# TencentYoutuResearch/ImageMatching-OETR

Measured on AMD Instinct MI355X. Metric: image-pairs/sec @640x640 (OETR hot path: feature correlation + overlap regression, features resident in HBM), higher is better.
Workload: dtype f32 (3xf16-split operands, fp32 accumulate); 1 GPU; BASELINE configs[1]: batch=8 pairs/GPU, 640x640 -> 20x20 tokens/image, C=256, 8 enc + 2 dec layers, f32_split_f16; pairs_per_gpu=8, global_pairs=8, streams=3, world_size=1, gpu_max_hw_queues=4, encoder_tile_rows=64, tail_mode=direct form (throughput setting for overlapped streams), parallelism=pairs sharded over 1 rank(s); all-gather of boxes only

## Files before the change

imagematching_oetr_amd/csrc/api.hip:

```cpp
#include <math.h>
#include <stdlib.h>
#include <string.h>

#include <string>
#include <vector>

#include "../../include/oetr_hip.h"
#include "common.h"

using namespace oetr;

constexpr int OETR_PREREDUCE_MIN_TOKENS = 768;
constexpr int OETR_DIRECT_TAIL_MIN_ROWS = 16000;

namespace {

thread_local std::string g_err;

oetr_status fail(oetr_status st, const std::string& msg) {
  g_err = msg;
  return st;
}
oetr_status hip_fail(hipError_t e, const char* what) {
  return fail(OETR_ERR_HIP, std::string(what) + ": " + hipGetErrorString(e));
// ... 96 lines not shown
  std::vector<int> kid;
  int used = 0;
  int dropped = 0;
};

struct oetr_ctx {
  oetr_trace* trace = nullptr;
  int device = 0;
  int mode = GM_SPLIT;
  int kv_prereduce = -1;
  mutable int dec_fault = 0;
  int dec_split = 0;
  int tail_mode = 0;
  int policy = 0;
  int enc_tile = 0;
  int attn_full = 0;
  int num_cus = 256;
  float* dev = nullptr;
  size_t dev_floats = 0;
  EncLayerDev enc[OETR_N_ENC];
  DecKVDev dkv;
  DecLayerDev dec[OETR_N_DEC];
  const float* qe[2];
  const float *dec_tgt1, *dec_q0, *dec_qkv1;
  HeadsDev heads;
};

struct oetr_neck_ctx {
  oetr_trace* trace = nullptr;
  int device = 0;
// ... 189 lines not shown

oetr_status run_correlation(oetr_ctx* h, const Geom& g, const Workspace& w, const float* feat1,
                            const float* feat2, const float* pos1, const float* pos2,
                            int enc_layers, hipStream_t s, bool with_decoder = true,
                            bool resident = false, const float* mask1 = nullptr,
                            const float* mask2 = nullptr) {
  EncLaunch p;
  memset(&p, 0, sizeof(p));
  if (!resident) {
    p.feat_nchw[0] = feat1; p.feat_nchw[1] = feat2;
    p.pos_nchw[0] = pos1; p.pos_nchw[1] = pos2;
    p.pos_out = w.pos;
  }
  p.tile_rows = encoder_tile_rows(h, g);
  p.g = encoder_geom(g, p.tile_rows);
#ifdef OETR_ABLATE
  { const char* e = getenv("OETR_ABLATE"); p.dbg = e ? atoi(e) : 0; }
#endif
#ifdef OETR_PHASE_TIMING
  {
    static long long* tb = nullptr;
    if (!tb) (void)hipMalloc(&tb, sizeof(long long) * 16 * 65536);
    p.tbuf = tb;
    g_tbuf = tb;
  }
#endif
  p.x = w.x; p.qp = w.qp; p.pos = w.pos;
  p.mask[0] = mask1; p.mask[1] = mask2;
  p.flags = w.flags;
  p.attn_full = h->attn_full;
// ... 959 lines not shown

void oetr_trace_destroy(oetr_trace_handle t) {
  if (!t) return;
  for (auto& e : t->ev) (void)hipEventDestroy(e);
  delete t;
}

oetr_status oetr_set_encoder_tile(oetr_handle h, int rows) {
  if (!h) return fail(OETR_ERR_BAD_ARG, "oetr_set_encoder_tile: NULL handle");
  if (rows != 0 && rows != TM && rows != 64)
    return fail(OETR_ERR_BAD_ARG, "oetr_set_encoder_tile: rows must be 0 (auto), 32 or 64");
  h->enc_tile = rows;
  return OETR_OK;
}

oetr_status oetr_set_tail_mode(oetr_handle h, int mode) {
  if (!h) return fail(OETR_ERR_BAD_ARG, "oetr_set_tail_mode: NULL handle");
  if (mode < 0 || mode > 3)
    return fail(OETR_ERR_BAD_ARG, "oetr_set_tail_mode: 0 (auto), 1 (P form), 2 (direct form) or 3 (direct form, per-tap staging)");
  if (mode >= 2 && h->mode != GM_SPLIT)
    return fail(OETR_ERR_UNSUPPORTED, "the direct 64-row heat-map conv is built for the two-plane dtypes (F32_SPLIT_F16, F32_SPLIT_QK16)");
  h->tail_mode = mode;
  return OETR_OK;
}

oetr_status oetr_set_decoder_split(oetr_handle h, int k) {
  if (!h) return fail(OETR_ERR_BAD_ARG, "oetr_set_decoder_split: NULL handle");
  if (k != 0 && k != 1 && k != DEC_SPLIT_K)
    return fail(OETR_ERR_BAD_ARG, "oetr_set_decoder_split: 0 (auto), 1 or 4 workgroups per image");
  h->dec_split = k;
// ... 87 lines not shown
```

imagematching_oetr_amd/csrc/common.h:

```cpp
#pragma once
#include <hip/hip_runtime.h>
#include <stdint.h>

#include <type_traits>

namespace oetr {

constexpr int C = 256;
constexpr int NH = 8;
constexpr int HD = 32;
constexpr int FF = 512;
constexpr int TM = 32;
constexpr int LDA = C + 4;
constexpr int LDH = FF + 4;
constexpr int NTHREADS = 256;
constexpr int KV_FLOATS = NH * HD * HD;
constexpr float LN_EPS = 1e-5f;
constexpr float ATTN_EPS = 1e-6f;
constexpr int MAX_TOKENS = 10000;


#ifdef OETR_ABLATE
#define ABL(flags, bit) (((flags) & (bit)) != 0)
#else
// ... 58 lines not shown
constexpr int LDAH = C + 8;
constexpr int LDHH = FF + 8;

struct Geom {
  int N;
  int L[2];
  int hf[2], wf[2];
  int nt[2];
  int row0[2];
  int prow0[2];
  int tile0[2];
  int ntiles;
  int rows;
};

#if defined(__HIPCC__)

__device__ __forceinline__ float wave_max(float v) {
#pragma unroll
  for (int off = 32; off > 0; off >>= 1) v = fmaxf(v, __shfl_xor(v, off, 64));
  return v;
}

__device__ __forceinline__ int crow(int r, int half) {
  return (r & 3) + 8 * (r >> 2) + 4 * half;
}

__device__ __forceinline__ float exp_neg(float x) {
  const float L2E_HI = 1.4426950216293335f, L2E_LO = 1.9259629911266175e-08f;
  const float t = x * L2E_HI;
// ... 724 lines not shown
  float* z0_out;
  float* dkv1_out;
  float* dks1_out;
  const float* dec_q0;
  EncLayerDev b;
  EncLayerDev a;
  DecKVDev d;
  int attn_full;
  const float* kbuf_in;
  const float* vt_in;
  float* kbuf_out;
  float* vt_out;
  int lpad[2];
  size_t vt_off[2];
  int tile_rows;
  int b_cross;
  int kv_reduced;
  int policy;
  int dbg;
  long long* tbuf;
  uint32_t* flags;
  const float* feat_nchw[2];
  const float* pos_nchw[2];
  float* pos_out;
  const float* mask[2];
};

hipError_t launch_encoder(const EncLaunch& p, bool has_b, int tail, int mode, hipStream_t s);
hipError_t launch_kv_reduce(const Geom& g, const float* kvp, const float* ksp, float* kvr, float* ksr,
                            hipStream_t s);
// ... 137 lines not shown
```

imagematching_oetr_amd/csrc/encoder.hip:

```cpp
#include <type_traits>

#include "common.h"


#ifndef OETR_SOAK_AMP
#define OETR_SOAK_AMP 0
#endif
#ifndef OETR_SPLIT_STATE
#define OETR_SPLIT_STATE 1
#endif

namespace oetr {

constexpr int S0_OFF = 0;
constexpr int S1_OFF = S0_OFF + TM * LDA;
constexpr int H_OFF = S1_OFF + TILE_FLOATS;
constexpr int KSUM_OFF = H_OFF + HID_FLOATS;
constexpr int Z_OFF = KSUM_OFF + C;
constexpr int LNP_OFF = Z_OFF + TM * NH;
constexpr int SMEM_FLOATS = LNP_OFF + 6 * C;

template <int NW>
struct EncCfg {
  static constexpr int NT = 8 / NW;
// ... 783 lines not shown
__device__ __forceinline__ void kv_state_write(const f32x16& kv, float ksum, int lane, int wave,
                                               float* __restrict__ kv_out,
                                               float* __restrict__ ks_out, int slot) {
  f32x4* dst = reinterpret_cast<f32x4*>(kv_out) + ((size_t)slot * NH + wave) * 4 * 64;
#pragma unroll
  for (int q = 0; q < 4; ++q) {
    f32x4 o = {kv[4 * q], kv[4 * q + 1], kv[4 * q + 2], kv[4 * q + 3]};
    store16(reinterpret_cast<float*>(dst), (q * 64 + (unsigned)lane) * 16u, o);
  }
  if (lane < 32) (ks_out + (size_t)slot * C + wave * HD)[(unsigned)lane] = ksum;
}

template <bool HAS_B, int TAIL, int MODE, int POL, int ROWS, int RTW = RT, bool MASKED = false>
__device__ __forceinline__ void encoder64_body(const EncLaunch& p, float* smem) {
  constexpr int NMT = RTW / 32, THREADS = 512, TPR = THREADS / RTW, F4 = 64 / TPR;
  using L2 = E2<RTW>;
  using SP = SitePolicy<POL>;
  float* R1f = smem + L2::R1;
  float* R2f = smem + L2::R2;
  Range rg;
  const PlanesT<MODE, RTW> P1(R1f, &rg), P2(R2f, &rg);
  float* Xf = HAS_B ? R2f : R1f;
  float* ksum_s = smem + L2::KSUM;
  float* lnp_s = smem + L2::LNP;
  float* lnx_s = smem + L2::LNX;
  using WS = WStream2T<MODE, ROWS, NMT>;
  WS ws;
  constexpr int P_MERGE = 0;
  constexpr int P_1A = WS::adv(P_MERGE), P_1B = WS::adv(P_1A), P_2A = WS::adv(P_1B), P_2B = WS::adv(P_2A);
  constexpr int P_T0 = HAS_B ? WS::adv(P_2B) : 0;
  constexpr int P_T1 = WS::adv(P_T0), P_T2 = WS::adv(P_T1), P_T3 = WS::adv(P_T2);

  const Geom& g = p.g;
  const int tid = threadIdx.x, lane = tid & 63, wave = __builtin_amdgcn_readfirstlane(tid >> 6);
  const int half = lane >> 5, col = lane & 31;
  const int wcol = 32 * wave;
  const int lrow = tid / TPR, lpart = tid % TPR;

  const int logical = xcd_remap(blockIdx.x, g.ntiles);
  const int per = g.nt[0] + g.nt[1];
  const int n = logical / per;
  const int rem = logical - n * per;
  const int side = rem >= g.nt[0];
  const int t_idx = side ? rem - g.nt[0] : rem;
  const int L = g.L[side];
  const int l0 = t_idx * RTW;
  const int nvalid = min(RTW, L - l0);
  const size_t row_base = (size_t)g.row0[side] + (size_t)n * L + l0;
  const int slot = g.tile0[side] + n * g.nt[side] + t_idx;
  const size_t qrow_base = (size_t)slot * RTW;
  const bool nchw = !HAS_B && p.feat_nchw[0] != nullptr;
  ws.set_rows(nvalid);
  ws.set_lane(lane);

  stage_ln_params<THREADS, HAS_B, TAIL>(lnp_s, p, tid);
  const f32x4* pos = reinterpret_cast<const f32x4*>(
                         p.pos + (size_t)(g.prow0[side] + l0 + min(lrow, nvalid - 1)) * C) + lpart;

  f32x16 xacc[NMT];
  PHASE_STAMP(p, 0);
  if (!HAS_B) PHASE_STAMP(p, 13);

  if (HAS_B) {
    const int ss = p.b_cross ? 1 - side : side;
    const int S_len = g.L[ss];
    const int nts = p.kv_reduced ? 1 : g.nt[ss];
    const int src_slot0 = p.kv_reduced ? ss * g.N + n : g.tile0[ss] + n * g.nt[ss];

    f32x4 kvB[4];
#pragma unroll
    for (int q = 0; q < 4; ++q) kvB[q] = f32x4{0.f, 0.f, 0.f, 0.f};
    {
      constexpr int KVR = 7;
      const unsigned ln = lane, kl = tid & (C - 1);
      const f32x4* kvp = reinterpret_cast<const f32x4*>(p.kv_in) + ((size_t)src_slot0 * NH + wave) * 256;
      const float* ksp = p.ks_in + (size_t)src_slot0 * C;
      float ks = 0.f;
      if (nts == 1) {
#pragma unroll
        for (int e = 0; e < 4; ++e) kvB[e] = kvp[e * 64 + ln];
        ks = ksp[kl];
      } else
      for (int ti0 = 0; ti0 < nts; ti0 += KVR) {
        f32x4 tmp[KVR][4];
        float kt[KVR];
#pragma unroll
        for (int u = 0; u < KVR; ++u) {
          const int ti = min(ti0 + u, nts - 1);
#pragma unroll
          for (int e = 0; e < 4; ++e) tmp[u][e] = kvp[(size_t)ti * (NH * 256) + e * 64 + ln];
          kt[u] = ksp[(size_t)ti * C + kl];
        }
#pragma unroll
        for (int u = 0; u < KVR; ++u)
          if (ti0 + u < nts) {
#pragma unroll
            for (int e = 0; e < 4; ++e) kvB[e] += tmp[u][e];
            ks += kt[u];
          }
      }
      if (tid < C) ksum_s[tid] = ks;
    }
    ws.template prime<C, P_MERGE, SP::MERGE>(p.b.wmerge, p.b.wmerge_l, wave, 0, lane);
    f32x4 qfrag[NMT][4];
    {
      const f32x4* qf = reinterpret_cast<const f32x4*>(p.qp + qrow_base * C) + (size_t)wave * NMT * 4 * 64;
#pragma unroll
      for (int mt = 0; mt < NMT; ++mt)
#pragma unroll
        for (int u = 0; u < 4; ++u) qfrag[mt][u] = qf[(mt * 4 + u) * 64 + (unsigned)lane];
    }
#pragma unroll
    for (int mt = 0; mt < NMT; ++mt) {
      const float* xr = p.x + (row_base + min(32 * mt + col, nvalid - 1)) * C + wcol + 4 * half;
#pragma unroll
      for (int g4 = 0; g4 < 4; ++g4) {
        const f32x4 v = *reinterpret_cast<const f32x4*>(xr + 8 * g4);
#pragma unroll
        for (int i = 0; i < 4; ++i) xacc[mt][4 * g4 + i] = v[i];
      }
    }
    __syncthreads();
    PHASE_STAMP(p, 1);

    {
      f32x4 kvh[2], kvl[2], ksh[2], ksl[2];
      const float inv_S = 1.0f / (float)S_len;
      (void)inv_S;
      if constexpr (gm_f16_range(MODE)) {
#pragma unroll
        for (int s2 = 0; s2 < 2; ++s2) {
          split8(kvB[2 * s2], kvB[2 * s2 + 1], kvh[s2], kvl[s2], rg);
          const float* kr = ksum_s + wave * HD + 4 * half + 16 * s2;
          split8(*reinterpret_cast<const f32x4*>(kr) * inv_S, *reinterpret_cast<const f32x4*>(kr + 8) * inv_S,
                 ksh[s2], ksl[s2], rg);
        }
      }
#pragma unroll
      for (int mt = 0; mt < NMT; ++mt) {
        if (mt == 1 && !ws.two()) break;
        f32x16 macc = {0}, zacc = {0};
        if constexpr (gm_f16_range(MODE)) {
          f32x16 c1 = {0}, cz = {0};
#pragma unroll
          for (int s2 = 0; s2 < 2; ++s2) {
            const f32x4 qh = qfrag[mt][2 * s2], ql = qfrag[mt][2 * s2 + 1];
            mma16_split3(kvh[s2], kvl[s2], qh, ql, macc, c1);
            mma16_split3(ksh[s2], ksl[s2], qh, ql, zacc, cz);
          }
#pragma unroll
          for (int r = 0; r < 16; ++r) macc[r] = fmaf(c1[r], SPLIT_INV, macc[r]);
          zacc[0] = fmaf(cz[0], SPLIT_INV, zacc[0]);
        } else {
#pragma unroll
          for (int ks4 = 0; ks4 < 4; ++ks4) {
            const f32x4 q = qfrag[mt][ks4];
            const f32x4 kk = *reinterpret_cast<const f32x4*>(ksum_s + wave * HD + 4 * half + ks4 * 8);
#pragma unroll
            for (int j = 0; j < 4; ++j) {
              macc = __builtin_amdgcn_mfma_f32_32x32x2f32(kvB[ks4][j], q[j], macc, 0, 0, 0);
              zacc = __builtin_amdgcn_mfma_f32_32x32x2f32(kk[j], q[j], zacc, 0, 0, 0);
            }
          }
        }
        const float zdot = gm_f16_range(MODE) ? zacc[0] * (float)S_len : zacc[0];
        const float zs = (float)S_len / (zdot + ATTN_EPS);
#pragma unroll
        for (int g4 = 0; g4 < 4; ++g4)
          P1.put4(32 * mt + col, wcol + 8 * g4 + 4 * half,
                  f32x4{macc[4 * g4] * zs, macc[4 * g4 + 1] * zs, macc[4 * g4 + 2] * zs, macc[4 * g4 + 3] * zs});
      }
    }
// ... 81 lines not shown
      PHASE_STAMP(p, 7);
      ws.template gemm<FF, P_2B, (TAIL != 2), C, SP::MLP2, SNEXT, XTR>(P1, p.b.w2, p.b.w2_l, wave, 16, lane, xacc,
                                                                       TAIL == 0 ? p.a.wq : p.d.wk[0],
                                                                       TAIL == 0 ? p.a.wq_l : p.d.wk_l[0], wave, 0);
    }
#pragma unroll
    for (int mt = 0; mt < NMT; ++mt)
#pragma unroll
      for (int g4 = 0; g4 < 4; ++g4)
        *reinterpret_cast<f32x4*>(Xf + (32 * mt + col) * LDA + wcol + 8 * g4 + 4 * half) =
            f32x4{xacc[mt][4 * g4], xacc[mt][4 * g4 + 1], xacc[mt][4 * g4 + 2], xacc[mt][4 * g4 + 3]};
    __syncthreads();
#pragma unroll
    for (int i = 0; i < RTW / 8; ++i) {
      const int r = wave + 8 * i;
      if (r < nvalid)
        store16(p.x + (row_base + r) * C, 16u * (unsigned)lane,
                                    *reinterpret_cast<const f32x4*>(Xf + r * LDA + 4 * lane));
    }
    PHASE_STAMP(p, 8);
    if (TAIL == 2) { range_report<MODE>(rg, p.flags); return; }
  } else {
    if (nchw) {
      load_tile_nchw<THREADS, RTW>(R1f, p.feat_nchw[side] + (size_t)n * C * L + l0, L, nvalid, tid);
      load_tile_nchw<THREADS, RTW>(R2f, p.pos_nchw[side] + l0, L, nvalid, tid);
    } else {
#pragma unroll
      for (int i = 0; i < (RTW * C / 4) / THREADS; ++i) {
        const int idx = tid + THREADS * i;
        const int r = idx >> 6, c4 = idx & 63;
        *reinterpret_cast<f32x4*>(R1f + r * LDA + 4 * c4) =
            reinterpret_cast<const f32x4*>(p.x + (row_base + min(r, nvalid - 1)) * C)[c4];
      }
    }
    if (TAIL == 0) ws.template prime<C, P_T0, SP::Q>(p.a.wq, p.a.wq_l, wave, 0, lane);
    if (TAIL == 1) ws.template prime<C, P_T0, SP::DEC_K>(p.d.wk[0], p.d.wk_l[0], wave, 0, lane);
    __syncthreads();
    if (nchw) {
      store_tile_tokens<THREADS, RTW>(p.x + row_base * C, R1f, nvalid, tid);
      if (n == 0) store_tile_tokens<THREADS, RTW>(p.pos_out + (size_t)(g.prow0[side] + l0) * C, R2f, nvalid, tid);
    }
    PHASE_STAMP(p, 14);
  }

  if constexpr (MASKED && TAIL != 2) {
    if (tid < RTW) lnx_s[tid] = tid < nvalid ? p.mask[side][(size_t)n * L + l0 + tid] : 0.f;
  }
  if (TAIL == 0) {
    {
      f32x4 xn[F4], ps[F4];
      if (!HAS_B && nchw) {
        const f32x4* pl = reinterpret_cast<const f32x4*>(R2f + lrow * LDA) + lpart;
#pragma unroll
        for (int i = 0; i < F4; ++i) ps[i] = pl[i * TPR];
      } else {
// ... 9 lines not shown
#pragma unroll
      for (int i = 0; i < F4; ++i) {
        P1.template put4<site_act_lo(SP::Q)>(lrow, 4 * (i * TPR + lpart), (xn[i] * qw[i * TPR] + qb[i * TPR]) + ps[i]);
        P2.template put4<site_act_lo(SP::K) || site_act_lo(SP::V)>(lrow, 4 * (i * TPR + lpart),
                                                                   (xn[i] * kw[i * TPR] + kb[i * TPR]) + ps[i]);
      }
    }
    __syncthreads();
    PHASE_STAMP(p, 9);
    f32x16 accQ[NMT] = {};
    ws.template gemm<C, P_T0, true, C, SP::Q, SP::K, true>(P1, p.a.wq, p.a.wq_l, wave, 0, lane, accQ, p.a.wk,
                                                           p.a.wk_l, wave, 0);
    PHASE_STAMP(p, 10);
    f32x16 accK[NMT] = {}, accV[NMT] = {};
    {
      f32x4* qf = reinterpret_cast<f32x4*>(p.qp + qrow_base * C) + (size_t)wave * NMT * 4 * 64;
      const bool two = ws.two();
      u32x4 qhi = {0, 0, 0, 0}, qlo = {0, 0, 0, 0};
      auto qepi = [&](auto CI_) {
        constexpr int CI = decltype(CI_)::value, mt = NMT == 2 ? CI / 8 : 0, pr = NMT == 2 ? CI % 8 : CI / 2;
        constexpr int s2 = pr / 4, j = pr % 4;
        if constexpr (NMT == 1 && CI % 2 == 1) return;
        if (mt == 1 && !two) return;
        const float qmask = MASKED ? lnx_s[32 * mt + col] : 1.0f;
        const float a = MASKED ? elu1(accQ[mt][2 * pr]) * qmask : elu1(accQ[mt][2 * pr]);
        const float b = MASKED ? elu1(accQ[mt][2 * pr + 1]) * qmask : elu1(accQ[mt][2 * pr + 1]);
        if constexpr (MODE == GM_BF16) {
          if constexpr (pr % 2 == 0) { qhi[0] = __builtin_bit_cast(uint32_t, a); qhi[1] = __builtin_bit_cast(uint32_t, b); }
          else {
            qhi[2] = __builtin_bit_cast(uint32_t, a); qhi[3] = __builtin_bit_cast(uint32_t, b);
            store16(reinterpret_cast<float*>(qf), ((mt * 4 + pr / 2) * 64 + (unsigned)lane) * 16u,
                                        __builtin_bit_cast(f32x4, qhi));
          }
        } else {
          uint32_t h, l;
          cvt_planes2<GM_SPLIT>(a, b, h, l, rg);
          qhi[j] = h; qlo[j] = l;
          if constexpr (j == 3) {
            store16(reinterpret_cast<float*>(qf), ((mt * 4 + 2 * s2) * 64 + (unsigned)lane) * 16u,
                                        __builtin_bit_cast(f32x4, qhi));
            store16(reinterpret_cast<float*>(qf), ((mt * 4 + 2 * s2 + 1) * 64 + (unsigned)lane) * 16u,
                                        __builtin_bit_cast(f32x4, qlo));
          }
        }
      };
      ws.template gemm_epi<C, P_T1, true, C, SP::K, SP::V>(P2, p.a.wk, p.a.wk_l, wave, 0, lane, accK, p.a.wv,
                                                           p.a.wv_l, wave, 0, qepi);
    }
    ws.template gemm<C, P_T2, false, C, SP::V>(P2, p.a.wv, p.a.wv_l, wave, 0, lane, accV, nullptr, nullptr,
                                               0, 0);
    PHASE_STAMP(p, 11);
    f32x16 kv;
    float ksum;
    kv_state_64<MODE, NMT, MASKED>(accK, accV, L, nvalid, half, ws.two(), kv, ksum, rg, lnx_s);
    kv_state_write(kv, ksum, lane, wave, p.kv_out, p.ks_out, slot);
    PHASE_STAMP(p, 12);
  } else if (TAIL == 1) {
    float bias_k[2], bias_v[2];
#pragma unroll
    for (int dl = 0; dl < 2; ++dl) {
      bias_k[dl] = p.d.bk[dl][wcol + col];
      bias_v[dl] = p.d.bv[dl][wcol + col];
    }
    {
      f32x4 xv[F4], ps[F4];
      const f32x4* src = reinterpret_cast<const f32x4*>(Xf + lrow * LDA) + lpart;
#pragma unroll
      for (int i = 0; i < F4; ++i) { xv[i] = src[i * TPR]; ps[i] = pos[i * TPR]; }
      __syncthreads();
#pragma unroll
// ... 3 lines not shown
      }
    }
    __syncthreads();
    auto dec_layer = [&](auto DL) {
      constexpr int dl = decltype(DL)::value;
      constexpr int PK = dl == 0 ? P_T0 : P_T2, PV = dl == 0 ? P_T1 : P_T3;
      f32x16 accK[NMT], accV[NMT];
#pragma unroll
      for (int mt = 0; mt < NMT; ++mt)
#pragma unroll
        for (int r = 0; r < 16; ++r) { accK[mt][r] = bias_k[dl]; accV[mt][r] = bias_v[dl]; }
      ws.template gemm<C, PK, true, C, SP::DEC_K, SP::DEC_V>(P1, p.d.wk[dl], p.d.wk_l[dl], wave, 0, lane, accK,
                                                             p.d.wv[dl], p.d.wv_l[dl], wave, 0);
      ws.template gemm<C, PV, false, C, SP::DEC_V>(P2, p.d.wv[dl], p.d.wv_l[dl], wave, 0, lane, accV, nullptr,
                                                   nullptr, 0, 0);
      f32x16 kv;
      float ksum;
      kv_state_64<MODE, NMT, MASKED>(accK, accV, L, nvalid, half, ws.two(), kv, ksum, rg, lnx_s);
      if constexpr (dl == 1) {
        kv_state_write(kv, ksum, lane, wave, p.dkv1_out, p.dks1_out, slot);
      } else {
        const float* q0 = p.dec_q0 + side * C + wave * HD;
        float a = 0.f;
#pragma unroll
        for (int r = 0; r < 16; ++r) a += q0[crow(r, half)] * kv[r];
        a += __shfl_xor(a, 32, 64);
        float z = q0[col] * ksum;
        z += __shfl_xor(z, 1, 64);
        z += __shfl_xor(z, 2, 64);
        z += __shfl_xor(z, 4, 64);
        z += __shfl_xor(z, 8, 64);
        z += __shfl_xor(z, 16, 64);
        if (half == 0) p.att0_out[(size_t)slot * C + wave * HD + col] = a;
        if (lane == 0) p.z0_out[(size_t)slot * NH + wave] = z;
        ws.template prime<C, P_T2, SP::DEC_K>(p.d.wk[1], p.d.wk_l[1], wave, 0, lane);
      }
    };
    dec_layer(std::integral_constant<int, 0>{});
    dec_layer(std::integral_constant<int, 1>{});
  }
  range_report<MODE>(rg, p.flags);
}

template <bool HAS_B, int TAIL, int MODE, int POL = 0, bool MASKED = false>
__global__ __launch_bounds__(512) void k_encoder64(EncLaunch p) {
  __shared__ __attribute__((aligned(16))) float smem[E2<RT>::SMEM];
  if constexpr (gm_planes(MODE) == 2) {
    const Geom& g = p.g;
    const int logical = xcd_remap(blockIdx.x, g.ntiles);
    const int per = g.nt[0] + g.nt[1];
    const int rem = logical - (logical / per) * per;
    const int side = rem >= g.nt[0];
    const int t_idx = side ? rem - g.nt[0] : rem;
    const int nvalid = min(RT, g.L[side] - t_idx * RT);
    if (__builtin_amdgcn_readfirstlane(nvalid > 32 ? 1 : 0)) encoder64_body<HAS_B, TAIL, MODE, POL, 2, RT, MASKED>(p, smem);
    else encoder64_body<HAS_B, TAIL, MODE, POL, 1, RT, MASKED>(p, smem);
  } else {
    encoder64_body<HAS_B, TAIL, MODE, POL, 0, RT, MASKED>(p, smem);
  }
}

template <bool HAS_B, int TAIL, int MODE, int POL = 0, bool MASKED = false>
__global__ __launch_bounds__(512) void k_encoder32m(EncLaunch p) {
  __shared__ __attribute__((aligned(16))) float smem[E2<TM>::SMEM];
  encoder64_body<HAS_B, TAIL, MODE, POL, 2, TM, MASKED>(p, smem);
}

template <int NOB_TAIL_MAX, class F>
static hipError_t launch_b_tail(bool has_b, int tail, F launch) {
  constexpr std::integral_constant<int, 0> t0{};
// ... 2 lines not shown
  if (has_b) {
    if (tail == 0) launch(std::true_type{}, t0);
    else if (tail == 1) launch(std::true_type{}, t1);
    else launch(std::true_type{}, t2);
  } else {
    if (tail == 0) launch(std::false_type{}, t0);
    else if constexpr (NOB_TAIL_MAX == 0) return hipErrorInvalidValue;
    else if (tail == 1) launch(std::false_type{}, t1);
    else if constexpr (NOB_TAIL_MAX == 1) return hipErrorInvalidValue;
    else launch(std::false_type{}, t2);
  }
  return hipGetLastError();
}

template <int MODE>
static hipError_t launch_encoder_mode(const EncLaunch& p, bool has_b, int tail, hipStream_t s) {
  const dim3 grid(p.g.ntiles);
  if (p.mask[0] || p.mask[1]) {
    if constexpr (MODE == GM_SPLIT) {
      if (!p.mask[0] || !p.mask[1] || (p.policy != 0 && p.policy != 1) || p.attn_full) return hipErrorInvalidValue;
      return launch_b_tail<0>(has_b, tail, [&](auto b, auto t) {
        if (p.policy == 1) {
          if (p.tile_rows == RT) hipLaunchKernelGGL((k_encoder64<b(), t(), MODE, 1, true>), grid, dim3(512), 0, s, p);
          else hipLaunchKernelGGL((k_encoder32m<b(), t(), MODE, 1, true>), grid, dim3(512), 0, s, p);
        } else {
          if (p.tile_rows == RT) hipLaunchKernelGGL((k_encoder64<b(), t(), MODE, 0, true>), grid, dim3(512), 0, s, p);
          else hipLaunchKernelGGL((k_encoder32m<b(), t(), MODE, 0, true>), grid, dim3(512), 0, s, p);
        }
      });
    } else if constexpr (MODE == GM_F32) {
      if (!p.mask[0] || !p.mask[1] || p.policy != 0 || p.attn_full) return hipErrorInvalidValue;
      return launch_b_tail<0>(has_b, tail, [&](auto b, auto t) {
// ... 99 lines not shown
```

imagematching_oetr_amd/hip_engine.py:

```python
import ctypes as C
import os
import time
from pathlib import Path

import torch

_PKG_DIR = Path(__file__).resolve().parent
LIB_PATH = _PKG_DIR / 'csrc' / 'liboetr_hip.so'

N_ENC, N_DEC, D_MODEL, N_HEAD = 8, 2, 256, 8
_f32p = C.POINTER(C.c_float)


class _EncW(C.Structure):
    _fields_ = [(n, _f32p) for n in (
        'q_proj', 'k_proj', 'v_proj', 'merge', 'mlp0', 'mlp2',
        'pre_norm_q_w', 'pre_norm_q_b', 'pre_norm_kv_w', 'pre_norm_kv_b',
        'norm2_w', 'norm2_b')]


class _MhaW(C.Structure):
    _fields_ = [(n, _f32p) for n in (
        'q_proj_w', 'q_proj_b', 'k_proj_w', 'k_proj_b', 'v_proj_w',
        'v_proj_b', 'merge')]
# ... 54 lines not shown
    'oetr_workspace_init', 'oetr_read_flags_async', 'oetr_neck_read_flags_async',
    'oetr_set_state_prereduce', 'oetr_set_tail_mode', 'oetr_set_decoder_split', 'oetr_overlap_frame', 'oetr_read_overlap_image',
    'oetr_forward_masked', 'oetr_feature_correlation_masked', 'oetr_center_estimation_masked',
    'oetr_linear_attention_masked', 'oetr_debug_decoder_fault',
    'oetr_flagslot_device_pointer', 'oetr_forward_flagslot', 'oetr_forward_tokens_flagslot',
    'oetr_neck_forward_tokens_status', 'oetr_debug_mfma_rate')

FLAG_F16_RANGE = 1
FLAG_EXCHANGE = 2
FLAG_INVALID = FLAG_F16_RANGE | FLAG_EXCHANGE
FLAG_PUBLISHED = 0x80000000

BANK_ABI_VERSION = 1
BANK_EXPORTS = ('oetr_bank_abi_version', 'oetr_bank_gather', 'oetr_forward_bank')
FLAG_INDEX = 4

COVIS_ABI_VERSION = 1
COVIS_EXPORTS = ('oetr_covis_abi_version', 'oetr_covis_workspace_bytes', 'oetr_covis_boxes')
COVIS_PARAM_DOUBLES = 40


def hot_path_keys():
    keys = []
    for i in range(N_ENC):
        p = f'transformer.encoder.{i}.'
        keys += [p + s for s in (
            'q_proj.weight', 'k_proj.weight', 'v_proj.weight', 'merge.weight',
            'mlp.0.weight', 'mlp.2.weight', 'pre_norm_q.weight',
            'pre_norm_q.bias', 'pre_norm_kv.weight', 'pre_norm_kv.bias',
            'norm2.weight', 'norm2.bias')]
# ... 151 lines not shown
    lib.oetr_overlap_frame.argtypes = [i, i, i, i] + [C.POINTER(i)] * 4 + [C.POINTER(C.c_double)] * 2
    lib.oetr_read_overlap_image.restype = i
    lib.oetr_read_overlap_image.argtypes = [vp, i, i, i, i, i, i, i, i, i, vp, vp, vp, vp]
    if lib.oetr_abi_version() != ABI_VERSION:
        raise RuntimeError(f'{p}: ABI version {lib.oetr_abi_version()} != '
                           f'{ABI_VERSION}')
    lib.oetr_bank_abi_version.restype = i
    lib.oetr_bank_abi_version.argtypes = []
    bank = [vp, i, vp, vp, i, vp, i]
    lib.oetr_bank_gather.restype = i
    lib.oetr_bank_gather.argtypes = bank + [i, i, vp, vp, vp, vp]
    lib.oetr_forward_bank.restype = i
    lib.oetr_forward_bank.argtypes = [vp] + bank + [i] * 8 + [vp, sz, vp, vp, vp, vp]
    if lib.oetr_bank_abi_version() != BANK_ABI_VERSION:
        raise RuntimeError(f'{p}: bank ABI version {lib.oetr_bank_abi_version()} != {BANK_ABI_VERSION}')
    lib.oetr_covis_abi_version.restype = i
    lib.oetr_covis_abi_version.argtypes = []
    lib.oetr_covis_workspace_bytes.restype = sz
    lib.oetr_covis_workspace_bytes.argtypes = [i]
    lib.oetr_covis_boxes.restype = i
    lib.oetr_covis_boxes.argtypes = [vp, vp, vp, i, i, i, vp, sz] + [vp] * 7
    if lib.oetr_covis_abi_version() != COVIS_ABI_VERSION:
        raise RuntimeError(f'{p}: covis ABI version {lib.oetr_covis_abi_version()} != {COVIS_ABI_VERSION}')
    if path is None:
        _lib = lib
    return lib


class OetrError(RuntimeError):
    pass
# ... 239 lines not shown
        if attention not in self.ATTENTIONS:
            raise ValueError(f'attention must be one of {sorted(self.ATTENTIONS)}')
        self.attention = attention
        if attention != 'linear':
            _check(self.lib, self.lib.oetr_set_attention(self._h, self.ATTENTIONS[attention]),
                   'oetr_set_attention')
        if os.environ.get('OETR_STATE_PREREDUCE'):
            self.set_state_prereduce(int(os.environ['OETR_STATE_PREREDUCE']))

    __del__ = _destructor('oetr_destroy')

    def set_encoder_tile(self, rows):
        _check(self.lib, self.lib.oetr_set_encoder_tile(self._h, int(rows or 0)),
               'oetr_set_encoder_tile')
        self._enc_tile_set = int(rows or 0)

    def _current_ws(self):
        return self._ws.get(torch.cuda.current_stream(self.device).cuda_stream)

    def set_state_prereduce(self, mode):
        _check(self.lib, self.lib.oetr_set_state_prereduce(self._h, int(mode)), 'oetr_set_state_prereduce')

    def set_tail_mode(self, mode):
        _check(self.lib, self.lib.oetr_set_tail_mode(self._h, int(mode)), 'oetr_set_tail_mode')
        self._tail_mode_set = int(mode)

    def set_decoder_split(self, k):
        _check(self.lib, self.lib.oetr_set_decoder_split(self._h, int(k)), 'oetr_set_decoder_split')
        self._dec_split_set = int(k)

# ... 600 lines not shown
```

Measured before the change: 33550 image-pairs/s.

## Pack both images' half-full encoder tail tiles into one mixed workgroup

When both images' last 64-row tiles hold at most 32 valid rows, the two half-tiles now run in one workgroup. A new mixed encoder body (ROWS==3) treats each 32-row half as an independent job, with its own side, slot, KV state and row bounds. This removes one workgroup per pair and keeps the other lanes of the tail tile busy. In exchange it adds a third template instantiation, more index arithmetic and a heavier per-workgroup path for the mixed tile. It is enabled by default only for unmasked, non-full-attention split-f16 runs with 64-row tiles.

```diff
diff --git a/imagematching_oetr_amd/csrc/api.hip b/imagematching_oetr_amd/csrc/api.hip
--- a/imagematching_oetr_amd/csrc/api.hip
+++ b/imagematching_oetr_amd/csrc/api.hip
@@ -6,6 +6,7 @@
 #include <vector>
 
 #include "../../include/oetr_hip.h"
+#include "../../include/oetr_tail_pairing.h"
 #include "common.h"
 
 using namespace oetr;
@@ -134,6 +135,7 @@
   int tail_mode = 0;
   int policy = 0;
   int enc_tile = 0;
+  int tail_pairing = -1;
   int attn_full = 0;
   int num_cus = 256;
   float* dev = nullptr;
@@ -353,6 +355,7 @@
   }
   p.tile_rows = encoder_tile_rows(h, g);
   p.g = encoder_geom(g, p.tile_rows);
+  p.pair_tails = h->tail_pairing != 0;
 #ifdef OETR_ABLATE
   { const char* e = getenv("OETR_ABLATE"); p.dbg = e ? atoi(e) : 0; }
 #endif
@@ -1342,6 +1345,34 @@
   return OETR_OK;
 }
 
+int oetr_tail_pairing_abi_version(void) { return OETR_TAIL_PAIRING_ABI_VERSION; }
+
+oetr_status oetr_set_encoder_tail_pairing(oetr_handle h, int mode) {
+  if (!h) return fail(OETR_ERR_BAD_ARG, "oetr_set_encoder_tail_pairing: NULL handle");
+  if (mode < -1 || mode > 1)
+    return fail(OETR_ERR_BAD_ARG, "oetr_set_encoder_tail_pairing: -1 (library rule), 0 (unpaired) or 1 (paired)");
+  h->tail_pairing = mode;
+  return OETR_OK;
+}
+
+oetr_status oetr_debug_encoder_jobs(int n_pairs, int L1, int L2, int pairing, int wg, int* n_workgroups, int* jobs) {
+  if (!n_workgroups || !jobs) return fail(OETR_ERR_BAD_ARG, "oetr_debug_encoder_jobs: NULL output");
+  if (n_pairs <= 0 || L1 <= 0 || L2 <= 0 || L1 > OETR_MAX_TOKENS || L2 > OETR_MAX_TOKENS)
+    return fail(OETR_ERR_BAD_SHAPE, "oetr_debug_encoder_jobs: invalid shape");
+  if (pairing < -1 || pairing > 1) return fail(OETR_ERR_BAD_ARG, "oetr_debug_encoder_jobs: pairing must be -1, 0 or 1");
+  const int nwg = n_pairs * enc_wg_per_pair(L1, L2, pairing);
+  *n_workgroups = nwg;
+  if (wg < 0 || wg >= nwg) return fail(OETR_ERR_BAD_ARG, "oetr_debug_encoder_jobs: workgroup outside the launch");
+  const EncWg w = enc_wg_jobs(wg, L1, L2, pairing);
+  jobs[0] = w.n; jobs[1] = w.mixed;
+  for (int j = 0; j < 2; ++j) {
+    jobs[2 + 2 * j] = w.side[j];
+    jobs[3 + 2 * j] = w.rt[j] < 0 ? -1 : 2 * w.tile[j] + w.rt[j];
+  }
+  jobs[6] = jobs[7] = 0;
+  return OETR_OK;
+}
+
 oetr_status oetr_set_tail_mode(oetr_handle h, int mode) {
   if (!h) return fail(OETR_ERR_BAD_ARG, "oetr_set_tail_mode: NULL handle");
   if (mode < 0 || mode > 3)
diff --git a/imagematching_oetr_amd/csrc/common.h b/imagematching_oetr_amd/csrc/common.h
--- a/imagematching_oetr_amd/csrc/common.h
+++ b/imagematching_oetr_amd/csrc/common.h
@@ -96,6 +96,49 @@
   int rows;
 };
 
+struct EncWg {
+  int n;
+  int side[2];
+  int tile[2];
+  int rt[2];
+  int mixed;
+};
+#if defined(__HIPCC__)
+#define OETR_HD __host__ __device__
+#else
+#define OETR_HD
+#endif
+OETR_HD inline bool enc_tail_is_half(int L) { return ((L - 1) & 63) < 32; }
+OETR_HD inline bool enc_pair_tails(int L0, int L1, int pairing) {
+  return pairing != 0 && enc_tail_is_half(L0) && enc_tail_is_half(L1);
+}
+OETR_HD inline int enc_wg_per_pair(int L0, int L1, int pairing) {
+  return (L0 + 63) / 64 + (L1 + 63) / 64 - (enc_pair_tails(L0, L1, pairing) ? 1 : 0);
+}
+OETR_HD inline EncWg enc_wg_jobs(int logical, int L0, int L1, int pairing) {
+  const int nt0 = (L0 + 63) / 64, nt1 = (L1 + 63) / 64;
+  const bool pair = enc_pair_tails(L0, L1, pairing);
+  const int per = nt0 + nt1 - (pair ? 1 : 0);
+  EncWg w;
+  w.n = logical / per;
+  const int rem = logical - w.n * per;
+  w.mixed = pair && rem == per - 1;
+  if (w.mixed) {
+    w.side[0] = 0; w.tile[0] = nt0 - 1; w.rt[0] = 0;
+    w.side[1] = 1; w.tile[1] = nt1 - 1; w.rt[1] = 0;
+    return w;
+  }
+  const int full0 = pair ? nt0 - 1 : nt0;
+  const int side = rem >= full0;
+  const int t = side ? rem - full0 : rem;
+  const int L = side ? L1 : L0;
+  w.side[0] = w.side[1] = side;
+  w.tile[0] = w.tile[1] = t;
+  w.rt[0] = 0;
+  w.rt[1] = L - 64 * t > 32 ? 1 : -1;
+  return w;
+}
+
 #if defined(__HIPCC__)
 
 __device__ __forceinline__ float wave_max(float v) {
@@ -850,6 +893,8 @@
   int lpad[2];
   size_t vt_off[2];
   int tile_rows;
+  int pair_tails;
+  int nwg;
   int b_cross;
   int kv_reduced;
   int policy;
diff --git a/imagematching_oetr_amd/csrc/encoder.hip b/imagematching_oetr_amd/csrc/encoder.hip
--- a/imagematching_oetr_amd/csrc/encoder.hip
+++ b/imagematching_oetr_amd/csrc/encoder.hip
@@ -821,6 +821,10 @@
 template <bool HAS_B, int TAIL, int MODE, int POL, int ROWS, int RTW = RT, bool MASKED = false>
 __device__ __forceinline__ void encoder64_body(const EncLaunch& p, float* smem) {
   constexpr int NMT = RTW / 32, THREADS = 512, TPR = THREADS / RTW, F4 = 64 / TPR;
+  constexpr bool MIX = ROWS == 3;
+  constexpr int NJ = MIX ? 2 : 1;
+  static_assert(!MIX || (RTW == RT && !MASKED && gm_planes(MODE) == 2), "the mixed body exists for the unmasked two-plane k_encoder64");
+  auto jt = [](int mt) { return MIX ? mt : 0; };
   using L2 = E2<RTW>;
   using SP = SitePolicy<POL>;
   float* R1f = smem + L2::R1;
@@ -831,7 +835,7 @@
   float* ksum_s = smem + L2::KSUM;
   float* lnp_s = smem + L2::LNP;
   float* lnx_s = smem + L2::LNX;
-  using WS = WStream2T<MODE, ROWS, NMT>;
+  using WS = WStream2T<MODE, MIX ? 2 : ROWS, NMT>;
   WS ws;
   constexpr int P_MERGE = 0;
   constexpr int P_1A = WS::adv(P_MERGE), P_1B = WS::adv(P_1A), P_2A = WS::adv(P_1B), P_2B = WS::adv(P_2A);
@@ -844,40 +848,72 @@
   const int wcol = 32 * wave;
   const int lrow = tid / TPR, lpart = tid % TPR;
 
-  const int logical = xcd_remap(blockIdx.x, g.ntiles);
-  const int per = g.nt[0] + g.nt[1];
-  const int n = logical / per;
-  const int rem = logical - n * per;
-  const int side = rem >= g.nt[0];
-  const int t_idx = side ? rem - g.nt[0] : rem;
-  const int L = g.L[side];
-  const int l0 = t_idx * RTW;
-  const int nvalid = min(RTW, L - l0);
-  const size_t row_base = (size_t)g.row0[side] + (size_t)n * L + l0;
-  const int slot = g.tile0[side] + n * g.nt[side] + t_idx;
-  const size_t qrow_base = (size_t)slot * RTW;
+  int n, side_j[NJ], L_j[NJ], l0_j[NJ], nvalid_j[NJ], slot_j[NJ];
+  size_t row_base_j[NJ];
+  if constexpr (RTW == RT) {
+    const EncWg wg = enc_wg_jobs(xcd_remap(blockIdx.x, p.nwg), g.L[0], g.L[1], p.pair_tails);
+    n = wg.n;
+#pragma unroll
+    for (int j = 0; j < NJ; ++j) {
+      side_j[j] = wg.side[j];
+      L_j[j] = g.L[side_j[j]];
+      l0_j[j] = wg.tile[j] * RTW;
+      slot_j[j] = g.tile0[side_j[j]] + n * g.nt[side_j[j]] + wg.tile[j];
+    }
+  } else {
+    const int logical = xcd_remap(blockIdx.x, g.ntiles);
+    const int per = g.nt[0] + g.nt[1];
+    n = logical / per;
+    const int rem = logical - n * per;
+    side_j[0] = rem >= g.nt[0];
+    const int t_idx = side_j[0] ? rem - g.nt[0] : rem;
+    L_j[0] = g.L[side_j[0]];
+    l0_j[0] = t_idx * RTW;
+    slot_j[0] = g.tile0[side_j[0]] + n * g.nt[side_j[0]] + t_idx;
+  }
+#pragma unroll
+  for (int j = 0; j < NJ; ++j) {
+    nvalid_j[j] = min(RTW, L_j[j] - l0_j[j]);
+    row_base_j[j] = (size_t)g.row0[side_j[j]] + (size_t)n * L_j[j] + l0_j[j];
+  }
+  const int side = side_j[0], L = L_j[0], l0 = l0_j[0], nvalid = nvalid_j[0], slot = slot_j[0];
+  const size_t row_base = row_base_j[0];
+  (void)side; (void)L; (void)l0; (void)slot;
+  auto xrow = [&](int mt, int r) -> size_t {
+    return MIX ? row_base_j[jt(mt)] + min(r, nvalid_j[jt(mt)] - 1) : row_base + min(32 * mt + r, nvalid - 1);
+  };
+  auto qfrag_ptr = [&](int mt) -> size_t {
+    return (size_t)slot_j[jt(mt)] * (RTW * C / 4) + ((size_t)wave * NMT + (MIX ? 0 : mt)) * 4 * 64;
+  };
   const bool nchw = !HAS_B && p.feat_nchw[0] != nullptr;
   ws.set_rows(nvalid);
   ws.set_lane(lane);
 
   stage_ln_params<THREADS, HAS_B, TAIL>(lnp_s, p, tid);
+  const bool jw = MIX && wave >= 4;
+  const int pos_row0 = jw ? g.prow0[side_j[NJ - 1]] + l0_j[NJ - 1] : g.prow0[side] + l0;
   const f32x4* pos = reinterpret_cast<const f32x4*>(
-                         p.pos + (size_t)(g.prow0[side] + l0 + min(lrow, nvalid - 1)) * C) + lpart;
+                         p.pos + (size_t)(pos_row0 + min(jw ? lrow - 32 : lrow, (jw ? nvalid_j[NJ - 1] : nvalid) - 1)) * C) + lpart;
 
   f32x16 xacc[NMT];
   PHASE_STAMP(p, 0);
   if (!HAS_B) PHASE_STAMP(p, 13);
 
   if (HAS_B) {
-    const int ss = p.b_cross ? 1 - side : side;
-    const int S_len = g.L[ss];
-    const int nts = p.kv_reduced ? 1 : g.nt[ss];
-    const int src_slot0 = p.kv_reduced ? ss * g.N + n : g.tile0[ss] + n * g.nt[ss];
-
-    f32x4 kvB[4];
-#pragma unroll
-    for (int q = 0; q < 4; ++q) kvB[q] = f32x4{0.f, 0.f, 0.f, 0.f};
-    {
+    int S_len_j[NJ];
+#pragma unroll
+    for (int j = 0; j < NJ; ++j) S_len_j[j] = g.L[p.b_cross ? 1 - side_j[j] : side_j[j]];
+
+    f32x4 kvB_j[NJ][4];
+#pragma unroll
+    for (int j = 0; j < NJ; ++j) {
+      f32x4 (&kvB)[4] = kvB_j[j];
+      const int ss = p.b_cross ? 1 - side_j[j] : side_j[j];
+      const int nts = p.kv_reduced ? 1 : g.nt[ss];
+      const int src_slot0 = p.kv_reduced ? ss * g.N + n : g.tile0[ss] + n * g.nt[ss];
+      float* ksum_d = j == 0 ? ksum_s : lnx_s;
+#pragma unroll
+      for (int q = 0; q < 4; ++q) kvB[q] = f32x4{0.f, 0.f, 0.f, 0.f};
       constexpr int KVR = 7;
       const unsigned ln = lane, kl = tid & (C - 1);
       const f32x4* kvp = reinterpret_cast<const f32x4*>(p.kv_in) + ((size_t)src_slot0 * NH + wave) * 256;
@@ -906,20 +942,21 @@
             ks += kt[u];
           }
       }
-      if (tid < C) ksum_s[tid] = ks;
+      if (tid < C) ksum_d[tid] = ks;
     }
     ws.template prime<C, P_MERGE, SP::MERGE>(p.b.wmerge, p.b.wmerge_l, wave, 0, lane);
     f32x4 qfrag[NMT][4];
     {
-      const f32x4* qf = reinterpret_cast<const f32x4*>(p.qp + qrow_base * C) + (size_t)wave * NMT * 4 * 64;
-#pragma unroll
-      for (int mt = 0; mt < NMT; ++mt)
-#pragma unroll
-        for (int u = 0; u < 4; ++u) qfrag[mt][u] = qf[(mt * 4 + u) * 64 + (unsigned)lane];
+#pragma unroll
+      for (int mt = 0; mt < NMT; ++mt) {
+        const f32x4* qf = reinterpret_cast<const f32x4*>(p.qp) + qfrag_ptr(mt);
+#pragma unroll
+        for (int u = 0; u < 4; ++u) qfrag[mt][u] = qf[u * 64 + (unsigned)lane];
+      }
     }
 #pragma unroll
     for (int mt = 0; mt < NMT; ++mt) {
-      const float* xr = p.x + (row_base + min(32 * mt + col, nvalid - 1)) * C + wcol + 4 * half;
+      const float* xr = p.x + xrow(mt, col) * C + wcol + 4 * half;
 #pragma unroll
       for (int g4 = 0; g4 < 4; ++g4) {
         const f32x4 v = *reinterpret_cast<const f32x4*>(xr + 8 * g4);
@@ -932,20 +969,27 @@
 
     {
       f32x4 kvh[2], kvl[2], ksh[2], ksl[2];
-      const float inv_S = 1.0f / (float)S_len;
-      (void)inv_S;
-      if constexpr (gm_f16_range(MODE)) {
-#pragma unroll
-        for (int s2 = 0; s2 < 2; ++s2) {
-          split8(kvB[2 * s2], kvB[2 * s2 + 1], kvh[s2], kvl[s2], rg);
-          const float* kr = ksum_s + wave * HD + 4 * half + 16 * s2;
-          split8(*reinterpret_cast<const f32x4*>(kr) * inv_S, *reinterpret_cast<const f32x4*>(kr + 8) * inv_S,
-                 ksh[s2], ksl[s2], rg);
-        }
-      }
+      auto state_frags = [&](int j) {
+        const float inv_S = 1.0f / (float)S_len_j[j];
+        (void)inv_S;
+        if constexpr (gm_f16_range(MODE)) {
+#pragma unroll
+          for (int s2 = 0; s2 < 2; ++s2) {
+            split8(kvB_j[j][2 * s2], kvB_j[j][2 * s2 + 1], kvh[s2], kvl[s2], rg);
+            const float* kr = (j == 0 ? ksum_s : lnx_s) + wave * HD + 4 * half + 16 * s2;
+            split8(*reinterpret_cast<const f32x4*>(kr) * inv_S, *reinterpret_cast<const f32x4*>(kr + 8) * inv_S,
+                   ksh[s2], ksl[s2], rg);
+          }
+        }
+      };
+      if constexpr (!MIX) state_frags(0);
 #pragma unroll
       for (int mt = 0; mt < NMT; ++mt) {
         if (mt == 1 && !ws.two()) break;
+        if constexpr (MIX) state_frags(mt);
+        const f32x4 (&kvB)[4] = kvB_j[jt(mt)];
+        const float* ksum_r = jt(mt) == 0 ? ksum_s : lnx_s;
+        const int S_len = S_len_j[jt(mt)];
         f32x16 macc = {0}, zacc = {0};
         if constexpr (gm_f16_range(MODE)) {
           f32x16 c1 = {0}, cz = {0};
@@ -962,7 +1006,7 @@
 #pragma unroll
           for (int ks4 = 0; ks4 < 4; ++ks4) {
             const f32x4 q = qfrag[mt][ks4];
-            const f32x4 kk = *reinterpret_cast<const f32x4*>(ksum_s + wave * HD + 4 * half + ks4 * 8);
+            const f32x4 kk = *reinterpret_cast<const f32x4*>(ksum_r + wave * HD + 4 * half + ks4 * 8);
 #pragma unroll
             for (int j = 0; j < 4; ++j) {
               macc = __builtin_amdgcn_mfma_f32_32x32x2f32(kvB[ks4][j], q[j], macc, 0, 0, 0);
@@ -1074,31 +1118,50 @@
 #pragma unroll
     for (int i = 0; i < RTW / 8; ++i) {
       const int r = wave + 8 * i;
-      if (r < nvalid)
-        store16(p.x + (row_base + r) * C, 16u * (unsigned)lane,
+      const int jr = MIX ? i / 4 : 0, rr = r - 32 * jr;
+      if (rr < nvalid_j[jr])
+        store16(p.x + (row_base_j[jr] + rr) * C, 16u * (unsigned)lane,
                                     *reinterpret_cast<const f32x4*>(Xf + r * LDA + 4 * lane));
     }
     PHASE_STAMP(p, 8);
     if (TAIL == 2) { range_report<MODE>(rg, p.flags); return; }
   } else {
     if (nchw) {
-      load_tile_nchw<THREADS, RTW>(R1f, p.feat_nchw[side] + (size_t)n * C * L + l0, L, nvalid, tid);
-      load_tile_nchw<THREADS, RTW>(R2f, p.pos_nchw[side] + l0, L, nvalid, tid);
+      if constexpr (MIX) {
+#pragma unroll
+        for (int j = 0; j < NJ; ++j) {
+          load_tile_nchw<THREADS, 32>(R1f + 32 * j * LDA, p.feat_nchw[side_j[j]] + (size_t)n * C * L_j[j] + l0_j[j],
+                                      L_j[j], nvalid_j[j], tid);
+          load_tile_nchw<THREADS, 32>(R2f + 32 * j * LDA, p.pos_nchw[side_j[j]] + l0_j[j], L_j[j], nvalid_j[j], tid);
+        }
+      } else {
+        load_tile_nchw<THREADS, RTW>(R1f, p.feat_nchw[side] + (size_t)n * C * L + l0, L, nvalid, tid);
+        load_tile_nchw<THREADS, RTW>(R2f, p.pos_nchw[side] + l0, L, nvalid, tid);
+      }
     } else {
 #pragma unroll
       for (int i = 0; i < (RTW * C / 4) / THREADS; ++i) {
         const int idx = tid + THREADS * i;
         const int r = idx >> 6, c4 = idx & 63;
         *reinterpret_cast<f32x4*>(R1f + r * LDA + 4 * c4) =
-            reinterpret_cast<const f32x4*>(p.x + (row_base + min(r, nvalid - 1)) * C)[c4];
+            reinterpret_cast<const f32x4*>(p.x + xrow(MIX ? i / 4 : 0, MIX ? r - 32 * (i / 4) : r) * C)[c4];
       }
     }
     if (TAIL == 0) ws.template prime<C, P_T0, SP::Q>(p.a.wq, p.a.wq_l, wave, 0, lane);
     if (TAIL == 1) ws.template prime<C, P_T0, SP::DEC_K>(p.d.wk[0], p.d.wk_l[0], wave, 0, lane);
     __syncthreads();
     if (nchw) {
-      store_tile_tokens<THREADS, RTW>(p.x + row_base * C, R1f, nvalid, tid);
-      if (n == 0) store_tile_tokens<THREADS, RTW>(p.pos_out + (size_t)(g.prow0[side] + l0) * C, R2f, nvalid, tid);
+      if constexpr (MIX) {
+#pragma unroll
+        for (int j = 0; j < NJ; ++j) {
+          store_tile_tokens<THREADS, 32>(p.x + row_base_j[j] * C, R1f + 32 * j * LDA, nvalid_j[j], tid);
+          if (n == 0) store_tile_tokens<THREADS, 32>(p.pos_out + (size_t)(g.prow0[side_j[j]] + l0_j[j]) * C,
+                                                     R2f + 32 * j * LDA, nvalid_j[j], tid);
+        }
+      } else {
+        store_tile_tokens<THREADS, RTW>(p.x + row_base * C, R1f, nvalid, tid);
+        if (n == 0) store_tile_tokens<THREADS, RTW>(p.pos_out + (size_t)(g.prow0[side] + l0) * C, R2f, nvalid, tid);
+      }
     }
     PHASE_STAMP(p, 14);
   }
@@ -1138,12 +1201,16 @@
     PHASE_STAMP(p, 10);
     f32x16 accK[NMT] = {}, accV[NMT] = {};
     {
-      f32x4* qf = reinterpret_cast<f32x4*>(p.qp + qrow_base * C) + (size_t)wave * NMT * 4 * 64;
+      f32x4* qf = reinterpret_cast<f32x4*>(p.qp) + qfrag_ptr(0);
+      f32x4* qf1 = MIX ? reinterpret_cast<f32x4*>(p.qp) + qfrag_ptr(NMT - 1) : qf;
+      (void)qf1;
       const bool two = ws.two();
       u32x4 qhi = {0, 0, 0, 0}, qlo = {0, 0, 0, 0};
       auto qepi = [&](auto CI_) {
         constexpr int CI = decltype(CI_)::value, mt = NMT == 2 ? CI / 8 : 0, pr = NMT == 2 ? CI % 8 : CI / 2;
         constexpr int s2 = pr / 4, j = pr % 4;
+        constexpr int mq = MIX ? 0 : mt;
+        f32x4* const qd = MIX && mt == 1 ? qf1 : qf;
         if constexpr (NMT == 1 && CI % 2 == 1) return;
         if (mt == 1 && !two) return;
         const float qmask = MASKED ? lnx_s[32 * mt + col] : 1.0f;
@@ -1153,7 +1220,7 @@
           if constexpr (pr % 2 == 0) { qhi[0] = __builtin_bit_cast(uint32_t, a); qhi[1] = __builtin_bit_cast(uint32_t, b); }
           else {
             qhi[2] = __builtin_bit_cast(uint32_t, a); qhi[3] = __builtin_bit_cast(uint32_t, b);
-            store16(reinterpret_cast<float*>(qf), ((mt * 4 + pr / 2) * 64 + (unsigned)lane) * 16u,
+            store16(reinterpret_cast<float*>(qd), ((mq * 4 + pr / 2) * 64 + (unsigned)lane) * 16u,
                                         __builtin_bit_cast(f32x4, qhi));
           }
         } else {
@@ -1161,9 +1228,9 @@
           cvt_planes2<GM_SPLIT>(a, b, h, l, rg);
           qhi[j] = h; qlo[j] = l;
           if constexpr (j == 3) {
-            store16(reinterpret_cast<float*>(qf), ((mt * 4 + 2 * s2) * 64 + (unsigned)lane) * 16u,
+            store16(reinterpret_cast<float*>(qd), ((mq * 4 + 2 * s2) * 64 + (unsigned)lane) * 16u,
                                         __builtin_bit_cast(f32x4, qhi));
-            store16(reinterpret_cast<float*>(qf), ((mt * 4 + 2 * s2 + 1) * 64 + (unsigned)lane) * 16u,
+            store16(reinterpret_cast<float*>(qd), ((mq * 4 + 2 * s2 + 1) * 64 + (unsigned)lane) * 16u,
                                         __builtin_bit_cast(f32x4, qlo));
           }
         }
@@ -1174,10 +1241,22 @@
     ws.template gemm<C, P_T2, false, C, SP::V>(P2, p.a.wv, p.a.wv_l, wave, 0, lane, accV, nullptr, nullptr,
                                                0, 0);
     PHASE_STAMP(p, 11);
-    f32x16 kv;
-    float ksum;
-    kv_state_64<MODE, NMT, MASKED>(accK, accV, L, nvalid, half, ws.two(), kv, ksum, rg, lnx_s);
-    kv_state_write(kv, ksum, lane, wave, p.kv_out, p.ks_out, slot);
+    if constexpr (MIX) {
+#pragma unroll
+      for (int j = 0; j < NJ; ++j) {
+        f32x16 kv;
+        float ksum;
+        kv_state_64<MODE, 1, MASKED>(reinterpret_cast<const f32x16(&)[1]>(accK[j]), reinterpret_cast<const f32x16(&)[1]>(accV[j]),
+                                     L_j[j], nvalid_j[j], half, false, kv, ksum, rg, lnx_s);
+        kv_state_write(kv, ksum, lane, wave, p.kv_out, p.ks_out, slot_j[j]);
+        asm volatile("" : "+v"(rg.fm));
+      }
+    } else {
+      f32x16 kv;
+      float ksum;
+      kv_state_64<MODE, NMT, MASKED>(accK, accV, L, nvalid, half, ws.two(), kv, ksum, rg, lnx_s);
+      kv_state_write(kv, ksum, lane, wave, p.kv_out, p.ks_out, slot);
+    }
     PHASE_STAMP(p, 12);
   } else if (TAIL == 1) {
     float bias_k[2], bias_v[2];
@@ -1211,13 +1290,20 @@
                                                              p.d.wv[dl], p.d.wv_l[dl], wave, 0);
       ws.template gemm<C, PV, false, C, SP::DEC_V>(P2, p.d.wv[dl], p.d.wv_l[dl], wave, 0, lane, accV, nullptr,
                                                    nullptr, 0, 0);
+#pragma unroll
+      for (int j = 0; j < NJ; ++j) {
       f32x16 kv;
       float ksum;
-      kv_state_64<MODE, NMT, MASKED>(accK, accV, L, nvalid, half, ws.two(), kv, ksum, rg, lnx_s);
+      if constexpr (MIX)
+        kv_state_64<MODE, 1, MASKED>(reinterpret_cast<const f32x16(&)[1]>(accK[j]), reinterpret_cast<const f32x16(&)[1]>(accV[j]),
+                                     L_j[j], nvalid_j[j], half, false, kv, ksum, rg, lnx_s);
+      else
+        kv_state_64<MODE, NMT, MASKED>(accK, accV, L, nvalid, half, ws.two(), kv, ksum, rg, lnx_s);
+      const int slot = slot_j[j];
       if constexpr (dl == 1) {
         kv_state_write(kv, ksum, lane, wave, p.dkv1_out, p.dks1_out, slot);
       } else {
-        const float* q0 = p.dec_q0 + side * C + wave * HD;
+        const float* q0 = p.dec_q0 + side_j[j] * C + wave * HD;
         float a = 0.f;
 #pragma unroll
         for (int r = 0; r < 16; ++r) a += q0[crow(r, half)] * kv[r];
@@ -1230,8 +1316,10 @@
         z += __shfl_xor(z, 16, 64);
         if (half == 0) p.att0_out[(size_t)slot * C + wave * HD + col] = a;
         if (lane == 0) p.z0_out[(size_t)slot * NH + wave] = z;
-        ws.template prime<C, P_T2, SP::DEC_K>(p.d.wk[1], p.d.wk_l[1], wave, 0, lane);
-      }
+      }
+      if constexpr (MIX) asm volatile("" : "+v"(rg.fm));
+      }
+      if constexpr (dl == 0) ws.template prime<C, P_T2, SP::DEC_K>(p.d.wk[1], p.d.wk_l[1], wave, 0, lane);
     };
     dec_layer(std::integral_constant<int, 0>{});
     dec_layer(std::integral_constant<int, 1>{});
@@ -1243,14 +1331,12 @@
 __global__ __launch_bounds__(512) void k_encoder64(EncLaunch p) {
   __shared__ __attribute__((aligned(16))) float smem[E2<RT>::SMEM];
   if constexpr (gm_planes(MODE) == 2) {
-    const Geom& g = p.g;
-    const int logical = xcd_remap(blockIdx.x, g.ntiles);
-    const int per = g.nt[0] + g.nt[1];
-    const int rem = logical - (logical / per) * per;
-    const int side = rem >= g.nt[0];
-    const int t_idx = side ? rem - g.nt[0] : rem;
-    const int nvalid = min(RT, g.L[side] - t_idx * RT);
-    if (__builtin_amdgcn_readfirstlane(nvalid > 32 ? 1 : 0)) encoder64_body<HAS_B, TAIL, MODE, POL, 2, RT, MASKED>(p, smem);
+    const EncWg wg = enc_wg_jobs(xcd_remap(blockIdx.x, p.nwg), p.g.L[0], p.g.L[1], p.pair_tails);
+    const int kind = __builtin_amdgcn_readfirstlane(wg.mixed ? 3 : wg.rt[1] >= 0 ? 2 : 1);
+    if constexpr (!MASKED) {
+      if (kind == 3) { encoder64_body<HAS_B, TAIL, MODE, POL, 3, RT, MASKED>(p, smem); return; }
+    }
+    if (kind == 2) encoder64_body<HAS_B, TAIL, MODE, POL, 2, RT, MASKED>(p, smem);
     else encoder64_body<HAS_B, TAIL, MODE, POL, 1, RT, MASKED>(p, smem);
   } else {
     encoder64_body<HAS_B, TAIL, MODE, POL, 0, RT, MASKED>(p, smem);
@@ -1283,8 +1369,12 @@
 }
 
 template <int MODE>
-static hipError_t launch_encoder_mode(const EncLaunch& p, bool has_b, int tail, hipStream_t s) {
-  const dim3 grid(p.g.ntiles);
+static hipError_t launch_encoder_mode(const EncLaunch& p_in, bool has_b, int tail, hipStream_t s) {
+  EncLaunch p = p_in;
+  p.pair_tails = (MODE == GM_SPLIT && p.pair_tails && p.tile_rows == RT && !p.mask[0] && !p.mask[1] && !p.attn_full &&
+                  enc_pair_tails(p.g.L[0], p.g.L[1], 1)) ? 1 : 0;
+  p.nwg = p.pair_tails ? p.g.N * enc_wg_per_pair(p.g.L[0], p.g.L[1], 1) : p.g.ntiles;
+  const dim3 grid(p.nwg);
   if (p.mask[0] || p.mask[1]) {
     if constexpr (MODE == GM_SPLIT) {
       if (!p.mask[0] || !p.mask[1] || (p.policy != 0 && p.policy != 1) || p.attn_full) return hipErrorInvalidValue;
diff --git a/imagematching_oetr_amd/hip_engine.py b/imagematching_oetr_amd/hip_engine.py
--- a/imagematching_oetr_amd/hip_engine.py
+++ b/imagematching_oetr_amd/hip_engine.py
@@ -92,6 +92,9 @@
 BANK_ABI_VERSION = 1
 BANK_EXPORTS = ('oetr_bank_abi_version', 'oetr_bank_gather', 'oetr_forward_bank')
 FLAG_INDEX = 4
+
+TAIL_PAIRING_ABI_VERSION = 1
+TAIL_PAIRING_EXPORTS = ('oetr_tail_pairing_abi_version', 'oetr_set_encoder_tail_pairing', 'oetr_debug_encoder_jobs')
 
 COVIS_ABI_VERSION = 1
 COVIS_EXPORTS = ('oetr_covis_abi_version', 'oetr_covis_workspace_bytes', 'oetr_covis_boxes')
@@ -273,6 +276,15 @@
     lib.oetr_forward_bank.argtypes = [vp] + bank + [i] * 8 + [vp, sz, vp, vp, vp, vp]
     if lib.oetr_bank_abi_version() != BANK_ABI_VERSION:
         raise RuntimeError(f'{p}: bank ABI version {lib.oetr_bank_abi_version()} != {BANK_ABI_VERSION}')
+    lib.oetr_tail_pairing_abi_version.restype = i
+    lib.oetr_tail_pairing_abi_version.argtypes = []
+    lib.oetr_set_encoder_tail_pairing.restype = i
+    lib.oetr_set_encoder_tail_pairing.argtypes = [vp, i]
+    lib.oetr_debug_encoder_jobs.restype = i
+    lib.oetr_debug_encoder_jobs.argtypes = [i, i, i, i, i, C.POINTER(i), C.POINTER(i)]
+    if lib.oetr_tail_pairing_abi_version() != TAIL_PAIRING_ABI_VERSION:
+        raise RuntimeError(f'{p}: tail-pairing ABI version {lib.oetr_tail_pairing_abi_version()} != '
+                           f'{TAIL_PAIRING_ABI_VERSION}')
     lib.oetr_covis_abi_version.restype = i
     lib.oetr_covis_abi_version.argtypes = []
     lib.oetr_covis_workspace_bytes.restype = sz
@@ -542,6 +554,10 @@
         _check(self.lib, self.lib.oetr_set_encoder_tile(self._h, int(rows or 0)),
                'oetr_set_encoder_tile')
         self._enc_tile_set = int(rows or 0)
+
+    def set_encoder_tail_pairing(self, mode):
+        _check(self.lib, self.lib.oetr_set_encoder_tail_pairing(self._h, int(mode)),
+               'oetr_set_encoder_tail_pairing')
 
     def _current_ws(self):
         return self._ws.get(torch.cuda.current_stream(self.device).cuda_stream)
diff --git a/include/oetr_tail_pairing.h b/include/oetr_tail_pairing.h
--- /dev/null
+++ b/include/oetr_tail_pairing.h
@@ -0,0 +1,22 @@
+#ifndef OETR_TAIL_PAIRING_H_
+#define OETR_TAIL_PAIRING_H_
+
+#include "oetr_hip.h"
+
+#ifdef __cplusplus
+extern "C" {
+#endif
+
+#define OETR_TAIL_PAIRING_ABI_VERSION 1
+
+int oetr_tail_pairing_abi_version(void);
+
+oetr_status oetr_set_encoder_tail_pairing(oetr_handle h, int mode);
+
+oetr_status oetr_debug_encoder_jobs(int n_pairs, int L1, int L2, int pairing, int wg,
+                                    int *n_workgroups, int *jobs);
+
+#ifdef __cplusplus
+}
+#endif
+#endif
```

Result: no change. 33420 image-pairs/s (-0.4%).
